# haotianteng/Chiron

Hardware: AMD Instinct MI355X
Metric: kilobases/sec basecalled (DNA_default seg_len=400 batch=1100) (higher is better)
Workload: dtype f32; 1 GPU; DNA_default seg_len=400 jump=390 batch=1100 greedy, synthetic 4 kHz signal (BASELINE.json configs[1]); segment_len=400, jump=390, batch=1100, decode=greedy, weights=seeded synthetic (exact checkpoint shapes), parallelism=reads sharded per GPU, no collective, slots_in_flight=3, parallelism_bookkeeping=none (one rank), distinct_devices=1

## Files before the change

chiron_amd/csrc/engine.hip:

```cpp
#include <hip/hip_runtime.h>

#include <algorithm>
#include <atomic>
#include <chrono>
#include <cfloat>
#include <cmath>
#include <cstdarg>
#include <cstdio>
#include <cstring>
#include <cstdlib>
#include <map>
#include <mutex>
#include <string>
#include <vector>

#include "../../include/chiron_amd.h"
#include "kernels.h"
#include "model_layout.h"
#include "weight_pack.h"
#include <dlfcn.h>

static const char* const kProfNames[] = {"conv_dma", "lstm_proj_dma", "lstm_recurrence", "fc_head", "ctc_greedy", "ctc_beam", "sparse_build",
                                         "path_prob", "conv_lift", "conv_res", "conv1_pwl", "conv_wino", "lstm_proj0_dma", "conv2a"};

// ... 63 lines not shown
};
struct CalibCtx {
  double* dev_sums = nullptr;
  size_t max_records = 0;
  std::vector<CalibRecord> rec;
  int skipped = 0;
};

struct ProfEvent {
  int name_id;
  hipEvent_t a, b;
  double flops, bytes;
};

struct Slot {
  hipStream_t stream = nullptr;
  unsigned long long* tile_ctr = nullptr;
  unsigned long long tile_base = 0;
  unsigned long long tile_base32 = 0;
  float* sig = nullptr;
  int32_t* seq = nullptr;
  float* act[5] = {nullptr, nullptr, nullptr, nullptr, nullptr};
  double* bn_sums = nullptr;
  float* z = nullptr;
  float* lasth[2] = {nullptr, nullptr};
  float* lasth_f32 = nullptr;
  float* logits = nullptr;
  uint8_t* labels = nullptr;
  int32_t* count = nullptr;
  float* log_prob = nullptr;
  float* prob = nullptr;
  int64_t* offsets = nullptr;
  int64_t* indices = nullptr;
  int64_t* values = nullptr;
  int64_t* meta = nullptr;
  void* beam_ws = nullptr;
  size_t beam_ws_bytes = 0;
  float* h_sig = nullptr;
  int32_t* h_seq = nullptr;
  int64_t* h_indices = nullptr;
  int64_t* h_values = nullptr;
  int64_t* h_meta = nullptr;
  float* h_log_prob = nullptr;
  float* h_prob = nullptr;
  float* h_logits = nullptr;
  uint8_t* h_labels = nullptr;
  int32_t* h_count = nullptr;
  uint8_t* h_flat = nullptr;
  struct State {
    std::atomic<int> v{0};
    State() {}
    State(const State& o) : v(o.v.load()) {}
    State& operator=(const State& o) {
      v.store(o.v.load());
      return *this;
    }
  } state;
  int batch = 0;
  uint32_t flags = 0;
  const float* sig_used = nullptr;
  int net_batch = 0;
  const float* rnn_out = nullptr;
  bool rnn_out_f32 = true;
  std::vector<ProfEvent> events;
  struct ScoreBufs {
    int32_t* labels = nullptr;
    int32_t* label_len = nullptr;
    float* loss = nullptr;
    float* edit = nullptr;
    int32_t* status = nullptr;
    uint64_t* ws = nullptr;
    size_t cap_labels = 0, cap_rows = 0, cap_ws = 0;
  } score;
};

struct chiron_engine : NetPlans {
  chiron_model_desc desc;
  BlobMap map;
  chiron_engine_opts opts;
  int L = 0, H = 0, K = 0;
  int maxB = 0, BP = 0;
  bool stream32 = true;
  bool stream16 = true;
  bool dyn_tiles = true;
  int lstm16_pair = -1;
  bool lstm16_fused = false;
  bool lstm16_narrow = false;
  bool lstm_fixed_roles = false;
  int lstm_form = 0;
  bool lstm_paired = false;
  bool bn_batch = false;
  bool f16 = false;
  bool w2 = false;
  bool lasth32 = true;
  bool w2_zf16 = false;
  bool split = false;
  int lasth_ld = 0;
  int kq = GEMM_BK;
  std::vector<Slot> slots;
  std::map<const float*, PlanHost> plan_host;
  std::vector<float> host_weights;
  CalibCtx* calib = nullptr;
  int calibrated = 0;
  std::vector<void*> owned;
  bool profiling = false;
  std::vector<std::string> prof_names;
  std::mutex mu;
};

static chiron_status dev_alloc(chiron_engine* e, void** p, size_t bytes, bool zero) {
  HIP_TRY(hipMalloc(p, bytes ? bytes : 16));
  e->owned.push_back(*p);
  if (zero) HIP_TRY(hipMemset(*p, 0, bytes ? bytes : 16));
  return CHIRON_OK;
}
static chiron_status upload_plans(chiron_engine* e, std::vector<Upload>& ups) {
  for (Upload& u : ups) {
    chiron_status st = dev_alloc(e, u.dst, u.bytes, false);
    if (st) return st;
    HIP_TRY(hipMemcpy(*u.dst, u.data, u.bytes, hipMemcpyHostToDevice));
    u.owner.reset();
    if (u.host.Npad > 0) e->plan_host[(const float*)*u.dst] = std::move(u.host);
  }
  return CHIRON_OK;
}

static bool split_row_scale() {
  static const bool on = getenv("CHIRON_SPLIT_NO_ROW_SCALE") == nullptr;
  return on;
}

static chiron_status build_plans(chiron_engine* e, const float* w) {
  e->bn_batch = e->desc.bn_mode == CHIRON_BN_BATCH;
  PackSwitches sw;
  sw.no_winograd = getenv("CHIRON_NO_WINOGRAD") != nullptr;
  sw.wino_f2 = getenv("CHIRON_WINOGRAD_F2") != nullptr;
  sw.wino_f4 = getenv("CHIRON_WINOGRAD_F4") != nullptr;
  sw.no_pwl = getenv("CHIRON_NO_PWL") != nullptr;
  sw.split_rec32 = getenv("CHIRON_SPLIT_REC32") != nullptr;
  if (e->split) sw.split_row_scale = split_row_scale();
  std::vector<Upload> ups;
  const chiron_status st = pack_weights(e->desc, e->map, w, e->L, e->opts.dtype, sw, e, &ups);
  return st ? st : upload_plans(e, ups);
}

static const uint64_t TENSOR_LIMIT = 0xFFFE0000ull;

static chiron_status plan_sizes(const chiron_model_desc* d, const chiron_engine_opts* o, chiron_engine_sizes* out) {
  BlobMap map;
  chiron_status st = blob_map(d, &map);
  if (st) return st;
  if (!o) return fail(CHIRON_ERR_INVALID, "null opts");
  if (o->max_batch < 1 || o->segment_len < 1) return fail(CHIRON_ERR_INVALID, "max_batch/segment_len must be positive");
  if (o->dtype != CHIRON_F32 && o->dtype != CHIRON_F16 && o->dtype != CHIRON_F32_SPLIT && o->dtype != CHIRON_F16_W2)
    return fail(CHIRON_ERR_INVALID, "dtype %d unknown (0 = f32, 1 = f16, 2 = f32 as hi/lo half pairs, 3 = f16 activations against hi/lo weights)", o->dtype);
  if (o->max_beam < 0) return fail(CHIRON_ERR_INVALID, "max_beam %d", o->max_beam);
  const bool f16 = o->dtype == CHIRON_F16 || o->dtype == CHIRON_F16_W2, split = o->dtype == CHIRON_F32_SPLIT, bn_batch = d->bn_mode == CHIRON_BN_BATCH;
  const uint64_t B = (uint64_t)o->max_batch, BP = (uint64_t)roundup(o->max_batch, 16), L = (uint64_t)o->segment_len, H = d->hidden, K = d->classes;
  SiteFrames fr[MAX_SITES];
  const uint64_t T = (uint64_t)frames(map, o->segment_len, fr);
  uint64_t tmax = 0, cmax = 0;
  for (int i = map.has_stem; i < map.n_sites; ++i) {
    tmax = std::max<uint64_t>(tmax, (uint64_t)std::max(fr[i].tin, fr[i].tout));
    cmax = std::max<uint64_t>(cmax, (uint64_t)map.site[i].co);
  }
  const uint64_t lasth_ld = !split ? 2 * H : d->rnn_kind == CHIRON_RNN_MULTI ? 2 * (uint64_t)roundup(d->hidden, 32) : (uint64_t)roundup(2 * d->hidden, 32);
  const uint64_t act = B * tmax * cmax * (f16 ? 2 : 4), lasth = T * BP * lasth_ld * 4, z = T * BP * 2 * 4 * H * 4;
  if (B * tmax >= (1ull << 31) || T * BP >= (1ull << 31))
    return fail(CHIRON_ERR_OVERFLOW, "max_batch %d x %llu frames does not fit the kernels' int row index", o->max_batch, (unsigned long long)tmax);
  if (act > TENSOR_LIMIT)
    return fail(CHIRON_ERR_OVERFLOW, "max_batch %d: an activation tensor [%d x %llu x %llu] needs %llu bytes, the kernels address at most %llu "
                "per tensor (about %llu windows at this segment length and dtype): use a smaller max_batch",
                o->max_batch, o->max_batch, (unsigned long long)tmax, (unsigned long long)cmax, (unsigned long long)act,
                (unsigned long long)TENSOR_LIMIT, (unsigned long long)(TENSOR_LIMIT / (tmax * cmax * (f16 ? 2 : 4))));
  if (T * BP * lasth_ld * (f16 ? 2 : 4) > TENSOR_LIMIT)
    return fail(CHIRON_ERR_OVERFLOW, "max_batch %d: the recurrent output [%llu x %llu x %llu] needs %llu bytes, the kernels address at most %llu per tensor",
                o->max_batch, (unsigned long long)T, (unsigned long long)BP, (unsigned long long)lasth_ld, (unsigned long long)lasth,
                (unsigned long long)TENSOR_LIMIT);
  uint64_t slot = B * L * 4 + BP * 4 + (bn_batch ? 5 : 3) * act + (bn_batch ? 2 * 2 * cmax * 8 : 0) + z + 2 * lasth + (split ? T * BP * 2 * H * 4 : 0);
  slot += B * T * K * 4 + B * T + 3 * B * 4 + (B + 1) * 8 + B * T * 16 + B * T * 8 + 3 * 8;
  if (o->max_beam > 0) slot += beam_workspace_bytes((int)B, (int)T, o->max_beam);
  if (out) {
    out->T = (int32_t)T;
    out->ratio = (double)o->segment_len / (double)T;
    out->largest_tensor_bytes = std::max(act, T * BP * lasth_ld * (f16 ? 2 : 4));
    out->tensor_limit_bytes = TENSOR_LIMIT;
    out->slot_bytes = slot;
    out->total_bytes = slot * (uint64_t)std::max(1, o->n_slots);
  }
  return CHIRON_OK;
}

extern "C" chiron_status chiron_engine_plan(const chiron_model_desc* desc, const chiron_engine_opts* opts, chiron_engine_sizes* out) {
  if (!out) return fail(CHIRON_ERR_INVALID, "null out");
  memset(out, 0, sizeof(*out));
  return plan_sizes(desc, opts, out);
}

static chiron_status alloc_slot(chiron_engine* e, Slot* s) {
  HIP_TRY(hipStreamCreateWithFlags(&s->stream, hipStreamNonBlocking));
  const size_t B = e->maxB, BP = e->BP, L = e->L, T = e->T, H = e->H, K = e->K;
  size_t tmax = 0, cmax = 0;
  for (const BlockPlan& b : e->blocks) {
    tmax = std::max<size_t>(tmax, b.t_in);
    tmax = std::max<size_t>(tmax, b.t_out);
    cmax = std::max<size_t>(cmax, b.c);
  }
  chiron_status st;
  if ((st = dev_alloc(e, (void**)&s->tile_ctr, 16 * sizeof(unsigned long long), true))) return st;
  if ((st = dev_alloc(e, (void**)&s->sig, B * L * 4, true))) return st;
  if ((st = dev_alloc(e, (void**)&s->seq, BP * 4, true))) return st;
  for (int i = 0; i < (e->bn_batch ? 5 : 3); ++i)
    if ((st = dev_alloc(e, (void**)&s->act[i], B * tmax * cmax * (e->f16 ? 2 : 4), false))) return st;
  if (e->bn_batch && (st = dev_alloc(e, (void**)&s->bn_sums, 2 * 2 * cmax * sizeof(double), true))) return st;
  if ((st = dev_alloc(e, (void**)&s->z, (size_t)T * BP * 2 * 4 * H * 4, true))) return st;
  for (int i = 0; i < 2; ++i)
    if ((st = dev_alloc(e, (void**)&s->lasth[i], T * BP * (size_t)e->lasth_ld * 4, true))) return st;
  if (e->split && (st = dev_alloc(e, (void**)&s->lasth_f32, T * BP * 2 * H * 4, true))) return st;
  if ((st = dev_alloc(e, (void**)&s->logits, B * T * K * 4, false))) return st;
  if ((st = dev_alloc(e, (void**)&s->labels, B * T, false))) return st;
  if ((st = dev_alloc(e, (void**)&s->count, B * 4, true))) return st;
  if ((st = dev_alloc(e, (void**)&s->log_prob, B * 4, true))) return st;
  if ((st = dev_alloc(e, (void**)&s->prob, B * 4, true))) return st;
  if ((st = dev_alloc(e, (void**)&s->offsets, (B + 1) * 8, true))) return st;
  if ((st = dev_alloc(e, (void**)&s->indices, B * T * 16, false))) return st;
  if ((st = dev_alloc(e, (void**)&s->values, B * T * 8, false))) return st;
  if ((st = dev_alloc(e, (void**)&s->meta, 3 * 8, true))) return st;
  if (e->opts.max_beam > 0) {
    s->beam_ws_bytes = beam_workspace_bytes((int)B, (int)T, e->opts.max_beam);
    if ((st = dev_alloc(e, &s->beam_ws, s->beam_ws_bytes, false))) return st;
  }
  HIP_TRY(hipHostMalloc((void**)&s->h_sig, B * L * 4, hipHostMallocDefault));
  HIP_TRY(hipHostMalloc((void**)&s->h_seq, BP * 4, hipHostMallocDefault));
  HIP_TRY(hipHostMalloc((void**)&s->h_indices, B * T * 16, hipHostMallocDefault));
  HIP_TRY(hipHostMalloc((void**)&s->h_values, B * T * 8, hipHostMallocDefault));
  HIP_TRY(hipHostMalloc((void**)&s->h_meta, 3 * 8, hipHostMallocDefault));
  HIP_TRY(hipHostMalloc((void**)&s->h_log_prob, B * 4, hipHostMallocDefault));
  HIP_TRY(hipHostMalloc((void**)&s->h_prob, B * 4, hipHostMallocDefault));
  HIP_TRY(hipHostMalloc((void**)&s->h_logits, B * T * K * 4, hipHostMallocDefault));
  HIP_TRY(hipHostMalloc((void**)&s->h_labels, B * T, hipHostMallocDefault));
  HIP_TRY(hipHostMalloc((void**)&s->h_count, B * 4, hipHostMallocDefault));
  s->h_flat = (uint8_t*)malloc(B * T ? B * T : 1);
  if (!s->h_flat) return fail(CHIRON_ERR_DEVICE, "out of host memory");
  memset(s->h_prob, 0, B * 4);
  return CHIRON_OK;
}

extern "C" chiron_status chiron_engine_create(const chiron_model_desc* desc, const float* weights, size_t n_floats,
                                              const chiron_engine_opts* opts, chiron_engine** out) {
  if (!out) return fail(CHIRON_ERR_INVALID, "null out");
  *out = nullptr;
  BlobMap map;
  chiron_status st = blob_map(desc, &map);
  if (st) return st;
  if (!weights || !opts) return fail(CHIRON_ERR_INVALID, "null weights/opts");
  if (map.total != n_floats) return fail(CHIRON_ERR_INVALID, "weight blob has %zu floats, descriptor needs %zu", n_floats, map.total);
  {
    chiron_engine_sizes sz;
    if ((st = plan_sizes(desc, opts, &sz))) return st;
  }
  if (desc->hidden != 100) return fail(CHIRON_ERR_INVALID, "hidden=%d: the recurrence kernel is built for hidden=100 (both shipped models)", desc->hidden);
  const bool trace = getenv("CHIRON_TRACE_CREATE") != nullptr;
  auto now = [] { return std::chrono::duration<double, std::milli>(std::chrono::steady_clock::now().time_since_epoch()).count(); };
  const double t_enter = now();
  int ndev = 0;
  if (hipGetDeviceCount(&ndev) != hipSuccess || ndev < 1) return fail(CHIRON_ERR_DEVICE, "no HIP device visible: libchiron_amd has no CPU fallback");
  if (opts->device_id < 0 || opts->device_id >= ndev) return fail(CHIRON_ERR_INVALID, "device_id %d out of range (%d devices)", opts->device_id, ndev);
  HIP_TRY(hipSetDevice(opts->device_id));
  if (trace) HIP_TRY(hipFree(nullptr));
  const double t_runtime = now();

  chiron_engine* e = new chiron_engine();
  e->desc = *desc;
  e->map = map;
  e->opts = *opts;
  if (e->opts.n_slots < 1) e->opts.n_slots = 1;
  e->L = opts->segment_len;
  e->H = desc->hidden;
  e->K = desc->classes;
  e->maxB = opts->max_batch;
  e->BP = roundup(opts->max_batch, 16);
  e->w2 = opts->dtype == CHIRON_F16_W2;
  e->w2_zf16 = e->w2 && getenv("CHIRON_W2_ZF16") != nullptr;
  e->lasth32 = getenv("CHIRON_F16_LASTH16") == nullptr;
  e->f16 = opts->dtype == CHIRON_F16 || e->w2;
  e->split = opts->dtype == CHIRON_F32_SPLIT;
  e->kq = e->f16 ? 2 * GEMM_BK : GEMM_BK;
  e->lasth_ld = !e->split ? 2 * desc->hidden
                : desc->rnn_kind == CHIRON_RNN_MULTI ? 2 * roundup(desc->hidden, 32) : roundup(2 * desc->hidden, 32);
  e->lstm_paired = getenv("CHIRON_LSTM_PAIR") != nullptr;
  e->lstm_fixed_roles = getenv("CHIRON_LSTM_FIXED_ROLES") != nullptr;
  {
    const char* wv = getenv("CHIRON_LSTM_WIDE");
    e->lstm_form = wv ? atoi(wv) : (e->split ? 0 : CHIRON_LSTM_WIDE_DEFAULT);
    if (e->lstm_form < 0 || e->lstm_form > 2) e->lstm_form = CHIRON_LSTM_WIDE_DEFAULT;
  }
  e->lstm16_narrow = getenv("CHIRON_LSTM16_NARROW") != nullptr;
  e->lstm16_pair = getenv("CHIRON_LSTM16_PAIR") ? atoi(getenv("CHIRON_LSTM16_PAIR")) : -1;
  e->stream16 = getenv("CHIRON_NO_STREAM16") == nullptr && opts->dtype != CHIRON_F16_W2;
  e->stream32 = getenv("CHIRON_NO_STREAM32") == nullptr;
  e->dyn_tiles = getenv("CHIRON_STATIC_TILES") == nullptr;
  {
    const int min_groups = getenv("CHIRON_LSTM16_FUSED_MIN") ? atoi(getenv("CHIRON_LSTM16_FUSED_MIN")) : 64;
    e->lstm16_fused = e->f16 && !e->w2 && !e->lstm16_narrow && desc->hidden == 100 && (e->BP / 16) * 2 >= min_groups && getenv("CHIRON_LSTM16_UNFUSED") == nullptr;
  }
  if (e->f16 && !e->w2) e->host_weights.assign(weights, weights + n_floats);
  st = build_plans(e, weights);
  const double t_plans = now();
  if (st == CHIRON_OK) {
    e->slots.resize(e->opts.n_slots);
    for (Slot& s : e->slots)
      if ((st = alloc_slot(e, &s))) break;
  }
  const double t_slots = now();
  if (st == CHIRON_OK && hipDeviceSynchronize() != hipSuccess) st = fail(CHIRON_ERR_DEVICE, "device sync after setup failed");
  if (trace)
    fprintf(stderr, "chiron_engine_create: {\"hip_runtime_and_context_ms\": %.1f, \"weights_prepared_and_uploaded_ms\": %.1f, \"slot_buffers_ms\": %.1f, "
                    "\"final_sync_ms\": %.1f, \"slots\": %d}\n", t_runtime - t_enter, t_plans - t_runtime, t_slots - t_plans, now() - t_slots, e->opts.n_slots);
  if (st) {
    chiron_engine_destroy(e);
    return st;
  }
  e->prof_names.assign(std::begin(kProfNames), std::end(kProfNames));
  *out = e;
  return CHIRON_OK;
}

extern "C" void chiron_engine_destroy(chiron_engine* e) {
  if (!e) return;
  hipSetDevice(e->opts.device_id);
  hipDeviceSynchronize();
  for (Slot& s : e->slots) {
    for (ProfEvent& ev : s.events) {
      hipEventDestroy(ev.a);
      hipEventDestroy(ev.b);
    }
    if (s.stream) hipStreamDestroy(s.stream);
    void* sp[] = {s.score.labels, s.score.label_len, s.score.loss, s.score.edit, s.score.status, s.score.ws};
    for (void* q : sp)
      if (q) hipFree(q);
    void* hp[] = {s.h_sig, s.h_seq, s.h_indices, s.h_values, s.h_meta, s.h_log_prob, s.h_prob, s.h_logits, s.h_labels, s.h_count};
    free(s.h_flat);
    for (void* q : hp)
      if (q) hipHostFree(q);
  }
  for (void* q : e->owned) hipFree(q);
  delete e;
}

extern "C" chiron_status chiron_engine_dims(const chiron_engine* e, int32_t* out_T, double* out_ratio) {
  if (!e) return fail(CHIRON_ERR_INVALID, "null engine");
  if (out_T) *out_T = e->T;
  if (out_ratio) *out_ratio = (double)e->L / (double)e->T;
  return CHIRON_OK;
}

enum { PN_CONV = 0, PN_PROJ, PN_REC, PN_FC, PN_GREEDY, PN_BEAM, PN_SPARSE, PN_PATHPROB, PN_LIFT, PN_RES, PN_PWL, PN_WINO, PN_PROJ0, PN_CONV2A };

struct Roctx {
  int (*push)(const char*) = nullptr;
  int (*pop)() = nullptr;
  Roctx() {
    const char* v = getenv("CHIRON_ROCTX");
    if (!v || !*v || *v == '0') return;
    for (const char* name : {"librocprofiler-sdk-roctx.so", "librocprofiler-sdk-roctx.so.1", "libroctx64.so", "libroctx64.so.4"}) {
      void* h = dlopen(name, RTLD_NOW | RTLD_GLOBAL);
      if (!h) continue;
      push = reinterpret_cast<int (*)(const char*)>(dlsym(h, "roctxRangePushA"));
      pop = reinterpret_cast<int (*)()>(dlsym(h, "roctxRangePop"));
      if (push && pop) return;
      push = nullptr, pop = nullptr;
    }
    fprintf(stderr, "chiron_amd: CHIRON_ROCTX is set but no roctx library could be loaded: no ranges\n");
  }
};
static const Roctx& roctx() {
  static const Roctx r;
  return r;
}

struct Prof {
  chiron_engine* e;
  Slot* s;
// ... 194 lines not shown
        done_pwl = launch_pwl_conv(q, s->stream);
      }
      if (!done_pwl) {
        {
          Prof pr(e, s, PN_LIFT, 2.0 * B * b.t_in * b.c, 4.0 * B * b.t_in + (e->f16 ? 2.0 : 4.0) * B * b.t_in * b.c);
          launch_lift(sig, b.lift_a, b.lift_b, bufA, (long)B * b.t_in, b.c, e->f16 ? 1 : e->split ? 2 : 0, s->stream);
        }
        GemmParams g = gemm_desc(e, b.gb, B, Mout, b.t_out, in_taps, 1, bufB, b.c);
        Prof pr(e, s, PN_CONV, 2.0 * B * b.t_out * (double)b.k * b.c * b.c, (e->f16 ? 2.0 : 4.0) * B * (b.t_in + b.t_out) * b.c);
        ok &= launch(e, g, s->stream);
      }
      GemmParams g = gemm_desc(e, b.gc, B, Mout, b.t_out, {GemmSeg{bufB, b.c, 0, b.c, cop, b.t_out, 1, 0, 0}}, 1, bufA, b.c);
      g.sig = sig;
      g.L = e->L;
      g.res_a = b.res_a;
      g.res_b = b.res_b;
      g.res_stride = b.stride;
      {
        Prof pr(e, s, PN_RES, 2.0 * B * b.t_out * (double)b.c * b.c, 8.0 * B * b.t_out * b.c);
        ok &= launch(e, g, s->stream);
      }
      x = bufA;
      xi = ia;
    } else {
      const int cip = roundup(b.c_in, e->kq);
      GemmParams g = gemm_desc(e, b.ga, B, (long)B * b.t_in, b.t_in, {GemmSeg{x, b.c_in, 0, b.c_in, cip, b.t_in, 1, 0, 0}}, 1, bufA, b.c);
      {
        Prof pr(e, s, PN_CONV2A, 2.0 * B * b.t_in * (double)b.c_in * b.c, 4.0 * B * b.t_in * (b.c_in + b.c));
        ok &= launch(e, g, s->stream);
      }
      g = gemm_desc(e, b.gb, B, Mout, b.t_out, in_taps, 1, bufB, b.c);
      {
        bool done = false;
        if (b.wino_u != nullptr) {
          WinoParams wq;
          wq.src = bufA, wq.U = b.wino_u, wq.shift = b.gb.shift, wq.out = bufB;
          wq.B = B, wq.T = b.t_in, wq.C = b.c, wq.N = b.c, wq.lda = b.c, wq.ldo = b.c, wq.relu = 1, wq.f4 = b.wino_f4;
          wq.tile_ctr = e->dyn_tiles ? s->tile_ctr : nullptr, wq.tile_base = 0, wq.tile_base_host = &s->tile_base;
          Prof pr(e, s, PN_WINO, 2.0 * B * b.t_out * (double)b.k * b.c * b.c, 4.0 * B * (b.t_in + b.t_out) * b.c);
          done = launch_wino_conv3(wq, s->stream);
        }
        if (!done) {
          Prof pr(e, s, PN_CONV, 2.0 * B * b.t_out * (double)b.k * b.c * b.c, 4.0 * B * (b.t_in + b.t_out) * b.c);
          ok &= launch(e, g, s->stream);
        }
      }
      g = gemm_desc(e, b.gc, B, Mout, b.t_out,
                    {GemmSeg{bufB, b.c, 0, b.c, cop, b.t_out, 1, 0, 0}, GemmSeg{x, b.c_in, 0, b.c_in, cip, b.t_in, b.stride, 0, 0}}, 1, bufA, b.c);
      {
        Prof pr(e, s, PN_CONV, 2.0 * B * b.t_out * (double)(b.c + b.c_in) * b.c, 4.0 * B * b.t_out * (2.0 * b.c + b.c_in));
        ok &= launch(e, g, s->stream);
      }
      x = bufA;
      xi = ia;
    }
  }
  s->sig_used = x;
  return ok;
}

static bool run_rnn(chiron_engine* e, Slot* s, int B) {
  bool ok = true;
  bool last_out_f32 = false;
  const float* fea = s->sig_used;
  const int T = e->T, H = e->H, BP = e->BP;
  const int zc = 4 * H;
  const float* prev = nullptr;
  for (size_t l = 0; l < e->lstm.size(); ++l) {
    const LstmPlan& lp = e->lstm[l];
    float* outbuf = s->lasth[l & 1];
    const bool fused = e->lstm16_fused && lp.wxwide != nullptr;
    for (int pj = 0; pj < (fused ? 0 : lp.nproj); ++pj) {
      const int Kp = roundup(lp.in_w, e->kq);
      const GemmSeg src = l == 0           ? GemmSeg{fea, e->C, 0, e->C, Kp, T, 1, 0, 0}
                          : lp.nproj == 1 ? GemmSeg{prev, e->lasth_ld, 0, 2 * H, Kp, T, 1, 0, 1}
                                          : GemmSeg{prev, e->lasth_ld, e->split ? pj * roundup(H, 32) : pj * H, H, Kp, T, 1, 0, 1};
      GemmParams g = gemm_desc(e, lp.proj[pj], B, (long)T * BP, T, {src}, 0, s->z, 0);
      g.m_time_major = 1;
      g.out_mode = 1;
      g.z_cols = zc;
      g.z_ndir = lp.nproj == 1 ? 2 : 1;
      g.z_dir0 = lp.nproj == 1 ? 0 : pj;
      g.z_seq_len = s->seq;
      g.z_f16 = (e->f16 && (!e->w2 || e->w2_zf16)) ? 1 : 0;
      const double ndir = lp.nproj == 1 ? 2.0 : 1.0;
      Prof pr(e, s, l == 0 ? PN_PROJ0 : PN_PROJ, 2.0 * B * T * (double)lp.in_w * 4 * H * ndir, 4.0 * B * T * (lp.in_w + ndir * zc));
      ok &= launch(e, g, s->stream);
    }
    LstmParams r;
    r.z = s->z;
    r.wfrag = lp.wfrag;
    r.wlight = lp.wlight;
    r.wwide = lp.wwide;
    r.wwide32 = lp.wwide32;
    r.wsplit = lp.wsplit;
    r.form32 = e->lstm_form;
    r.narrow16 = e->lstm16_narrow ? 1 : 0;
    r.xsrc = nullptr;
    r.wxwide = nullptr;
    r.whfused = nullptr;
    r.fused_pair = 0;
    r.xbias = nullptr;
    r.xK = r.xld = r.x_time_major = 0;
    if (fused) {
      r.xsrc = l == 0 ? (const void*)fea : (const void*)prev;
      r.wxwide = lp.wxwide;
      r.whfused = lp.whfused;
      r.fused_pair = e->lstm16_pair >= 0 ? (e->lstm16_pair ? 1 : 0) : ((BP / 16) * 2 > current_device_cus() ? 1 : 0);
      r.xbias = lp.proj[0].shift;
      r.xK = lp.in_w;
      r.xld = l == 0 ? e->C : e->lasth_ld;
      r.x_time_major = l == 0 ? 0 : 1;
    }
    r.seq_len = s->seq;
    r.out = e->split ? s->lasth_f32 : outbuf;
    r.out_f32 = (e->f16 && e->lasth32 && e->calib == nullptr && l + 1 == e->lstm.size()) ? 1 : 0;
    last_out_f32 = r.out_f32 != 0;
    const bool direct_split = e->split && lp.wsplit != nullptr && l + 1 < e->lstm.size();
    r.out_split = direct_split ? (void*)outbuf : nullptr;
    r.split_ld = e->lasth_ld;
    r.split_bw0 = e->desc.rnn_kind == CHIRON_RNN_MULTI ? roundup(H, 32) : H;
    r.T = T;
    r.B = B;
    r.BP = BP;
    r.H = H;
    r.ndir = 2;
    r.paired = e->lstm_paired ? 1 : 0;
    r.fixed_roles = e->lstm_fixed_roles ? 1 : 0;
    r.group0 = 0;
    r.f16 = e->f16 ? 1 : 0;
    r.w2 = e->w2 ? (e->w2_zf16 ? 2 : 1) : 0;
    if (e->calib && e->f16) {
      for (int pj = 0; pj < lp.nproj; ++pj) {
        const int dir = lp.nproj == 1 ? -1 : pj;
        if (l == 0)
          calib_measure(e, lp.proj[pj].shift, 0, fea, (long)B * T, e->C, 0, e->C, 0, B, (int)l, dir, 0, s->stream);
        else
          calib_measure(e, lp.proj[pj].shift, 0, prev, (long)T * BP, e->lasth_ld, lp.nproj == 1 ? 0 : pj * H, lp.in_w, BP, B, (int)l, dir, 0, s->stream);
      }
    }
    {
      Prof pr(e, s, PN_REC, 2.0 * 2.0 * B * T * (double)H * 4 * H + (fused ? 2.0 * B * T * (double)lp.in_w * 4 * H * 2.0 : 0.0),
              fused ? (e->f16 ? 2.0 : 4.0) * B * T * (2.0 * lp.in_w + 2.0 * H) : 4.0 * B * T * 2.0 * (zc + H));
      launch_lstm(r, s->stream);
    }
    if (e->calib && e->f16)
      for (int dir = 0; dir < 2; ++dir)
        calib_measure(e, lp.proj[lp.nproj == 1 ? 0 : dir].shift, 0, outbuf, (long)T * BP, e->lasth_ld, dir * H, H, BP, B, (int)l, dir, 1, s->stream);
    prev = outbuf;
    if (e->split) {
      if (direct_split) {
      } else if (l + 1 < e->lstm.size()) {
        Prof pr(e, s, PN_REC, 0.0, (4.0 + 4.0) * T * BP * 2.0 * H);
        const bool multi = e->desc.rnn_kind == CHIRON_RNN_MULTI;
        launch_split_convert(s->lasth_f32, outbuf, (long)T * BP, 2 * H, e->lasth_ld, multi ? H : 0, multi ? roundup(H, 32) : 0, s->stream);
      } else {
        prev = s->lasth_f32;
      }
    }
  }
  s->rnn_out = prev;
  FcParams f;
  f.lasth = prev;
  f.w = e->fc_w;
  f.bias = e->fc_b;
  f.wc = e->fc_wc;
// ... 582 lines not shown
```

chiron_amd/csrc/gemm.hip:

```cpp
#include "kernels.h"
#include "timing_variants.h"

#include <cstdlib>
#include <type_traits>

namespace chiron {

typedef float f32x16 __attribute__((ext_vector_type(16)));
typedef float f32x4 __attribute__((ext_vector_type(4)));
typedef _Float16 f16x8 __attribute__((ext_vector_type(8)));
typedef _Float16 f16x4 __attribute__((ext_vector_type(4)));

constexpr int LDS_LD = GEMM_BK + 4;
constexpr int TILE_F = GEMM_BM * LDS_LD;

struct ZGroup {
  unsigned base;
  unsigned per_t;
  int t, l0, l1, l2, l3;
  __device__ __forceinline__ ZGroup(const GemmParams& p, int t_, int b) : t(t_) {
    per_t = (unsigned)(p.BP >> 2) * p.z_dirs_total * p.z_cols * 4;
    base = (unsigned)(b >> 2) * p.z_dirs_total * p.z_cols * 4;
    const int4 len = *reinterpret_cast<const int4*>(p.z_seq_len + b);
    l0 = min(len.x, p.T_out), l1 = min(len.y, p.T_out), l2 = min(len.z, p.T_out), l3 = min(len.w, p.T_out);
// ... 826 lines not shown
#pragma unroll
              for (int j = 0; j < 4; ++j)
                if (g * 4 + j < NP) piece(g * 4 + j);
              continue;
            }
            f32x4 a[NMI], b[NNI];
#pragma unroll
            for (int mi = 0; mi < NMI; ++mi) a[mi] = *reinterpret_cast<const f32x4*>(a0 + mi * 32 * GEMM_BK + fsl(g));
#pragma unroll
            for (int ni = 0; ni < NNI; ++ni) b[ni] = *reinterpret_cast<const f32x4*>(b0 + ni * 32 * GEMM_BK + fsl(g));
            if (F16) {
#pragma unroll
              for (int j = 0; j < 4; ++j)
                if (g * 4 + j < NP) piece(g * 4 + j);
#pragma unroll
              for (int mi = 0; mi < NMI; ++mi)
#pragma unroll
                for (int ni = 0; ni < NNI; ++ni) {
                  const f32x16 c = acc[mi][ni];
                  const f16x8 ah = __builtin_bit_cast(f16x8, a[mi]), bh = __builtin_bit_cast(f16x8, b[ni]);
                  acc[mi][ni] = ZOUT ? __builtin_amdgcn_mfma_f32_32x32x16_f16(ah, bh, c, 0, 0, 0)
                                     : __builtin_amdgcn_mfma_f32_32x32x16_f16(bh, ah, c, 0, 0, 0);
                }
            } else {
#pragma unroll
              for (int j = 0; j < 4; ++j) {
                if (g * 4 + j < NP) piece(g * 4 + j);
#pragma unroll
                for (int mi = 0; mi < NMI; ++mi)
#pragma unroll
                  for (int ni = 0; ni < NNI; ++ni) {
                    const f32x16 c = acc[mi][ni];
#if CHIRON_SENS & 16
                    if (j & 1) { acc[mi][ni][0] += a[mi][j] * b[ni][j]; continue; }
#endif
                    acc[mi][ni] = ZOUT ? __builtin_amdgcn_mfma_f32_32x32x2f32(a[mi][j], b[ni][j], c, 0, 0, 0)
                                       : __builtin_amdgcn_mfma_f32_32x32x2f32(b[ni][j], a[mi][j], c, 0, 0, 0);
                  }
              }
#if CHIRON_SENS & 4096
              if (ZOUT && FS && have_prev && C * 4 + g < 4 * NNI) {
                const int sq = (C * 4 + g) / NNI, sni = (C * 4 + g) % NNI;
                const unsigned gstr = (unsigned)p.z_dirs_total * p.z_cols * 4;
                float* o = p.out + (unsigned)((pm0 + wave * 32 + 8 * sq + 4 * kh) >> 2) * gstr + (unsigned)(p.z_dir0 * p.z_cols + pn0 + li) * 4 + sni * 128;
                if (pm0 + wave * 32 + 8 * sq + 4 * kh < p.M) *reinterpret_cast<f32x4*>(o) = a[0];
              }
#endif
            }
          }
          }
        }
        buf ^= 1;
      };
      chunk(std::integral_constant<int, 0>{});
      if (CPS > 1) chunk(std::integral_constant<int, 1>{});
      if (CPS > 2) chunk(std::integral_constant<int, 2>{});
      if (CPS > 3) chunk(std::integral_constant<int, 3>{});
      if (CPS > 4) chunk(std::integral_constant<int, 4>{});
      if (CPS > 5) chunk(std::integral_constant<int, 5>{});
      if (CPS > 6) chunk(std::integral_constant<int, 6>{});
      if (CPS > 7) chunk(std::integral_constant<int, 7>{});
    };
    segment(std::true_type{}, 0);
    for (int sgi = 1; sgi < nseg; ++sgi) segment(std::false_type{}, sgi);

    have_prev = true;
    pm0 = m0;
    pn0 = n0;
    c_id = n_id;
#if CHIRON_SENS & 1024
    ++clk_tiles;
#endif
  }
  if (have_prev) epilogue(pm0, pn0);
#if CHIRON_SENS & 1024
  if (tid == 0 && blockIdx.x < 4 && clk_tiles > 0)
    printf("gemm_clk zout %d K %d block %d: tiles %llu, cycles per tile: total %llu, epilogue %llu, barriers %llu %llu %llu %llu %llu %llu %llu %llu\n",
           (int)ZOUT, p.K, (int)blockIdx.x, clk_tiles, (__builtin_amdgcn_s_memtime() - clk_t0) / clk_tiles, clk_epi / clk_tiles, clk_bar[0] / clk_tiles,
           clk_bar[1] / clk_tiles, clk_bar[2] / clk_tiles, clk_bar[3] / clk_tiles, clk_bar[4] / clk_tiles, clk_bar[5] / clk_tiles, clk_bar[6] / clk_tiles,
           clk_bar[7] / clk_tiles);
#endif
}

template <bool ZOUT, bool RES>
static bool launch_dma(const GemmParams& p, dim3 grid, dim3 block, hipStream_t stream) {
  const int kpad = p.seg[0].kpad, cin = p.seg[0].cin;
  constexpr int BN = ZOUT ? 160 : GEMM_BN;
  if (((p.N + BN - 1) / BN) * BN > DMA_MAX_N) return false;
  if (ZOUT && p.z_cols < BN) return false;
  for (int s = 1; s < p.nseg; ++s)
    if (p.seg[s].kpad != kpad || p.seg[s].cin != cin) return false;
  const bool tail = cin != kpad;
  if (p.f16 == 2) {
    if (!ZOUT && p.N % GEMM_BN) return false;
    if constexpr (ZOUT) {
      if (p.nseg == 1 && kpad == 256 && !tail) {
        hipLaunchKernelGGL((gemm_f32_dma_kernel<true, false, 8, false, 2, true>), grid, block, 0, stream, p);
        return true;
      }
      if (p.nseg == 1 && kpad == 224 && tail) {
        hipLaunchKernelGGL((gemm_f32_dma_kernel<true, false, 7, true, 2, true>), grid, block, 0, stream, p);
        return true;
      }
    }
    if (kpad == 256 && !tail) {
      hipLaunchKernelGGL((gemm_f32_dma_kernel<ZOUT, RES, 8, false, 2>), grid, block, 0, stream, p);
      return true;
    }
    if constexpr (ZOUT) {
      if (kpad == 224 && tail) {
        hipLaunchKernelGGL((gemm_f32_dma_kernel<true, false, 7, true, 2>), grid, block, 0, stream, p);
        return true;
      }
      if (kpad == 128 && tail) {
        hipLaunchKernelGGL((gemm_f32_dma_kernel<true, false, 4, true, 2>), grid, block, 0, stream, p);
        return true;
      }
    }
    return false;
  }
  if (p.f16) {
    if (!ZOUT && p.N % GEMM_BN) return false;
    if (kpad == 128 && !tail) {
      hipLaunchKernelGGL((gemm_f32_dma_kernel<ZOUT, RES, 4, false, 1>), grid, block, 0, stream, p);
      return true;
    }
    if constexpr (ZOUT) {
      if (kpad == 128 && tail) {
        hipLaunchKernelGGL((gemm_f32_dma_kernel<true, false, 4, true, 1>), grid, block, 0, stream, p);
        return true;
      }
      if (kpad == 64 && tail) {
        hipLaunchKernelGGL((gemm_f32_dma_kernel<true, false, 2, true, 1>), grid, block, 0, stream, p);
        return true;
      }
    }
    return false;
  }
  if constexpr (ZOUT) {
    if (p.nseg == 1) {
      if (kpad == 256 && !tail) {
        hipLaunchKernelGGL((gemm_f32_dma_kernel<true, false, 8, false, 0, true>), grid, block, 0, stream, p);
        return true;
      }
      if (kpad == 224 && tail) {
        hipLaunchKernelGGL((gemm_f32_dma_kernel<true, false, 7, true, 0, true>), grid, block, 0, stream, p);
        return true;
      }
    }
  }
  if (kpad == 256 && !tail) {
    hipLaunchKernelGGL((gemm_f32_dma_kernel<ZOUT, RES, 8, false>), grid, block, 0, stream, p);
    return true;
  }
  if constexpr (ZOUT) {
    if (kpad == 224 && tail) {
      hipLaunchKernelGGL((gemm_f32_dma_kernel<true, false, 7, true>), grid, block, 0, stream, p);
      return true;
    }
    if (kpad == 128 && tail) {
      hipLaunchKernelGGL((gemm_f32_dma_kernel<true, false, 4, true>), grid, block, 0, stream, p);
      return true;
    }
  }
  return false;
}

bool launch_gemm(const GemmParams& p0, hipStream_t stream) {
  GemmParams p = p0;
  const int nblocks_n = (p.N + GEMM_BN - 1) / GEMM_BN;
  const int mblocks = (p.M + GEMM_BM - 1) / GEMM_BM;
  const int total_ids = ((mblocks + 7) / 8) * 8 * nblocks_n;
  const int n_cu = current_device_cus();
  static const int wgs_per_cu = [] {
    const char* v = getenv("CHIRON_GEMM_WGS_PER_CU");
    const int n = v ? atoi(v) : 2;
    return n >= 1 && n <= 8 ? n : 2;
  }();
  int g = wgs_per_cu * n_cu;
  g = (g / 8) * 8;
  if (g > total_ids) g = total_ids;
  const dim3 grid(g), block(256);
  const int total_z = ((mblocks + 7) / 8) * 8 * ((p.N + 159) / 160);
  const dim3 grid_z(std::min((wgs_per_cu * n_cu / 8) * 8, total_z));
  const bool zout = p.out_mode == 1;
  const bool dyn = p.tile_ctr != nullptr && p.tile_base_host != nullptr && p.seg[0].src != nullptr && p.seg[0].kpad / GEMM_BK >= 3 &&
                   (zout ? grid_z.x : grid.x) % 8 == 0;
  if (dyn) p.tile_base = *p.tile_base_host;
  else p.tile_ctr = nullptr;
  auto advance = [&](bool launched) {
    if (launched && dyn) *p.tile_base_host += (unsigned long long)((zout ? total_z : total_ids) / 8 + (zout ? grid_z.x : grid.x) / 8);
    return launched;
  };
  if (p.f16) {
    if (p.seg[0].src == nullptr) return false;
    if (p.out_mode == 1) return advance(launch_dma<true, false>(p, grid_z, block, stream));
    if (p.res_a != nullptr) return advance(launch_dma<false, true>(p, grid, block, stream));
    return advance(launch_dma<false, false>(p, grid, block, stream));
  }
  if (p.seg[0].src == nullptr) {
    hipLaunchKernelGGL((gemm_f32_kernel<true, false, false>), grid, block, 0, stream, p);
  } else if (p.out_mode == 1) {
    if (!advance(launch_dma<true, false>(p, grid_z, block, stream)))
      hipLaunchKernelGGL((gemm_f32_kernel<false, true, false>), grid, block, 0, stream, p);
  } else if (p.res_a != nullptr) {
    if (!advance(launch_dma<false, true>(p, grid, block, stream)))
      hipLaunchKernelGGL((gemm_f32_kernel<false, false, true>), grid, block, 0, stream, p);
  } else {
    if (!advance(launch_dma<false, false>(p, grid, block, stream)))
      hipLaunchKernelGGL((gemm_f32_kernel<false, false, false>), grid, block, 0, stream, p);
  }
  return true;
}

}
```

chiron_amd/csrc/kernels.h:

```cpp
#pragma once
#include <hip/hip_runtime.h>
#include <stdint.h>

#include "../../include/chiron_amd.h"

#define CHIRON_KMAX 5

namespace chiron {

constexpr int CHIRON_MAX_DEVICES = 64;
inline int current_device_index() {
  int dev = 0;
  if (hipGetDevice(&dev) != hipSuccess || dev < 0 || dev >= CHIRON_MAX_DEVICES) dev = 0;
  return dev;
}
inline int current_device_cus() {
  static int n_cu[CHIRON_MAX_DEVICES] = {};
  const int dev = current_device_index();
  int n = __atomic_load_n(&n_cu[dev], __ATOMIC_RELAXED);
  if (n == 0) {
    hipDeviceProp_t prop;
    n = hipGetDeviceProperties(&prop, dev) == hipSuccess ? prop.multiProcessorCount : 0;
    if (n <= 0) n = 256;
    __atomic_store_n(&n_cu[dev], n, __ATOMIC_RELAXED);
  }
  return n;
}

constexpr int GEMM_MAX_SEG = 16;
constexpr int GEMM_BM = 128;
constexpr int GEMM_BN = 128;
constexpr int GEMM_BK = 32;

struct GemmSeg {
  const float* src;
  int lda;
  int col0;
  int cin;
  int kpad;
  int w_in;
  int stride;
  int shift;
  int time_major;
};

struct GemmParams {
  int M;
  int T_out;
  int B;
  int BP;
  int m_time_major;
  int N;
  int K;
  int nseg;
  GemmSeg seg[GEMM_MAX_SEG];
  const float* Wt;
  const float* shift;
  const float* descale;
  int relu;
  const float* sig;
  int L;
  const float* lift_a;
  const float* lift_b;
  const float* res_a;
  const float* res_b;
  int res_stride;
  float* out;
  int ldo;
  int out_mode;
  int z_cols;
  int z_ndir;
  int z_dir0;
  int z_dirs_total;
  const int32_t* z_seq_len;
  int f16;
  int z_f16;
  unsigned long long* tile_ctr;
  unsigned long long tile_base;
  unsigned long long* tile_base_host;
};

bool launch_gemm(const GemmParams& p, hipStream_t stream);
bool launch_stream16(const GemmParams& p, hipStream_t stream);
bool launch_stream32(const GemmParams& p, hipStream_t stream);


struct WinoParams {
  const float* src;
  const float* U;
  const float* shift;
  float* out;
  int B, T, C, N, lda, ldo, relu;
  int f4;
  unsigned long long* tile_ctr;
  unsigned long long tile_base;
  unsigned long long* tile_base_host;
};
bool launch_wino_conv3(const WinoParams& p, hipStream_t stream);

constexpr int LSTM_K = 100;
constexpr int LSTM_NW = 7;

struct LstmParams {
  const float* z;
  const float* wfrag;
  const float* wlight;
  const float* wwide32;
  int out_f32;
  const void* wsplit;
  void* out_split;
  int split_ld;
  int split_bw0;
  int form32;
  const void* wwide;
  const void* xsrc;
  const void* wxwide;
  const void* whfused;
  int fused_pair;
  const float* xbias;
  int xK, xld, x_time_major;
  const int32_t* seq_len;
  float* out;
  int T, B, BP, H;
  int ndir;
  int paired;
  int fixed_roles;
  int group0;
  int narrow16;
  int w2;
  int f16;
};
void launch_lstm(const LstmParams& p, hipStream_t stream);
constexpr int LSTM_KSTEPS16 = 25;

void launch_stem_conv(const float* sig, const float* w, const float* shift, void* out, int B, int L, int T_out, int k, int stride, int left,
                      int C, int fmt, int relu, hipStream_t stream);
void launch_split_convert(const float* src, void* dst, long rows, int cols, int ld, int half, int half_dst, hipStream_t stream);
struct PwlConvParams {
  const float* sig;
  const float* bp;
  const float* ref;
// ... 193 lines not shown
```

chiron_amd/csrc/weight_pack.h:

```cpp
#pragma once
#include <algorithm>
#include <cfloat>
#include <cmath>
#include <memory>
#include <utility>
#include <vector>

#include "kernels.h"
#include "model_layout.h"

namespace chiron {

inline int roundup(int v, int m) { return (v + m - 1) / m * m; }

struct ConvGemmPlan {
  float* Wt = nullptr;
  float* shift = nullptr;
  float* descale = nullptr;
  int N = 0, Npad = 0, K = 0;
};

struct PlanHost {
  std::vector<float> dW;
  std::vector<float> shift0;
  int N = 0, Npad = 0, K = 0;
};

struct BlockPlan {
  bool lift = false;
  int c_in = 0, c = 0, k = 0, stride = 1, left = 0;
  int t_in = 0, t_out = 0;
  float *lift_a = nullptr, *lift_b = nullptr;
  float *res_a = nullptr, *res_b = nullptr;
  float *pwl_bp = nullptr, *pwl_ref = nullptr, *pwl_tab = nullptr, *pwl_shift = nullptr;
  int pwl_nbp = 0;
  ConvGemmPlan ga, gb, gc;
  float* wino_u = nullptr;
  int wino_f4 = 0;
  ConvGemmPlan g1;
  bool i_bn = false;
  float *bn_scale[4] = {nullptr, nullptr, nullptr, nullptr}, *bn_offset[4] = {nullptr, nullptr, nullptr, nullptr};
};

struct LstmPlan {
  int in_w = 0;
  ConvGemmPlan proj[2];
  int nproj = 1;
  float* wfrag = nullptr;
  void* wwide = nullptr;
  void* whfused = nullptr;
  void* wxwide = nullptr;
  int wx_ksteps = 0;
  void* wsplit = nullptr;
  float* wwide32 = nullptr;
  float* wlight = nullptr;
};

struct NetPlans {
  int T = 0, C = 0;
  int stem_k = 0, stem_stride = 1, stem_left = 0, stem_t = 0, stem_c = 0;
  float *stem_w = nullptr, *stem_shift = nullptr, *stem_scale = nullptr, *stem_offset = nullptr;
  std::vector<BlockPlan> blocks;
  std::vector<LstmPlan> lstm;
  float *fc_w = nullptr, *fc_b = nullptr, *fc_wc = nullptr, *fc_bc = nullptr;
};

struct PackSwitches {
  bool no_winograd = false;
  bool wino_f2 = false;
  bool wino_f4 = false;
  bool no_pwl = false;
  bool split_rec32 = false;
  bool split_row_scale = true;
};

struct Upload {
  void** dst;
  std::shared_ptr<void> owner;
  const void* data;
  size_t bytes;
  PlanHost host;
};


struct HalfPair {
  _Float16 hi, lo;
};
inline HalfPair split_half(float v) {
  const _Float16 hi = (_Float16)v;
  return {hi, (_Float16)(v - (float)hi)};
}

struct BnFold {
  std::vector<float> inv, sh;
};
inline BnFold fold_bn(const float* scale, const float* offset, const float* mean, const float* var, int n) {
  BnFold f;
  f.inv.resize(n);
  f.sh.resize(n);
  for (int i = 0; i < n; ++i) {
    const float inv = (1.0f / sqrtf(var[i] + 1e-5f)) * scale[i];
    f.inv[i] = inv;
    f.sh[i] = offset[i] - mean[i] * inv;
  }
  return f;
}

inline void fold_filter(std::vector<float>& Wt, std::vector<float>& shift, int K, int k0, const float* W, int taps, int ci, int co, int cop,
                        const float* inv, const float* sh) {
  for (int n = 0; n < co; ++n) {
    for (int tap = 0; tap < taps; ++tap)
      for (int c = 0; c < ci; ++c) {
        const float v = W[((size_t)tap * ci + c) * co + n];
        Wt[(size_t)n * K + k0 + tap * cop + c] = inv ? v * inv[n] : v;
      }
    if (sh) shift[n] = k0 == 0 ? sh[n] : shift[n] + sh[n];
  }
}

struct LstmKernels {
  const float* kern[2];
  int H;
  float at(int dir, int k_off, int width, int k, int g, int unit) const {
    return k < width && unit < H ? kern[dir][(size_t)(k_off + k) * 4 * H + g * H + unit] : 0.f;
  }
};

template <class Put>
inline void narrow_fragments(const LstmKernels& kn, int V, int ksteps, int k_off, int width, Put put) {
  for (int dir = 0; dir < 2; ++dir)
    for (int wv = 0; wv < LSTM_NW; ++wv)
      for (int ks = 0; ks < ksteps; ++ks)
        for (int lane = 0; lane < 64; ++lane)
          for (int q = 0; q < V; ++q) {
            const int k = V * ks + q, g = lane >> 4, unit = 16 * wv + (lane & 15);
            put(((((size_t)dir * LSTM_NW + wv) * ksteps + ks) * 64 + lane) * V + q, kn.at(dir, k_off, width, k, g, unit));
          }
}
inline size_t narrow_elems(int V, int ksteps) { return (size_t)2 * LSTM_NW * ksteps * 64 * V; }

template <class Put>
inline void wide_fragments(const LstmKernels& kn, int V, int ksteps, int k_off, int width, Put put) {
  for (int dir = 0; dir < 2; ++dir)
    for (int wv = 0; wv < 8; ++wv)
      for (int slot = 0; slot < (wv == 7 ? 4 : 3); ++slot)
        for (int ks = 0; ks < ksteps; ++ks)
          for (int lane = 0; lane < 64; ++lane)
            for (int q = 0; q < V; ++q) {
              const int k = V * (4 * ks + (lane >> 4)) + q, g = lane & 3, unit = 4 * (3 * wv + slot) + ((lane >> 2) & 3);
              put((((((size_t)dir * 8 + wv) * 4 + slot) * ksteps + ks) * 64 + lane) * V + q, kn.at(dir, k_off, width, k, g, unit));
            }
}
inline size_t wide_elems(int V, int ksteps) { return (size_t)2 * 8 * 4 * ksteps * 64 * V; }

inline std::vector<float> light_fragment(const LstmKernels& kn, int k_off) {
  std::vector<float> wl((size_t)2 * 28 * 64, 0.f);
  for (int dir = 0; dir < 2; ++dir)
    for (int m = 0; m < 28; ++m)
      for (int lane = 0; lane < 64; ++lane) {
        const int q = m >> 2, a = m & 3, kg = lane >> 4, g = (lane >> 2) & 3, j = lane & 3;
        const int k = 16 * q + 4 * kg + a;
        wl[((size_t)dir * 28 + m) * 64 + lane] = kn.at(dir, k_off, kn.H, k, g, 96 + j);
      }
  return wl;
}

struct WeightPacker {
  const chiron_model_desc& d;
  const BlobMap& map;
  const float* w;
  const PackSwitches sw;
  const bool f16, w2, split, batch;
  const int kq;
// ... 328 lines not shown
```

Baseline: 4582 kbases/s.

## Run fp32 LSTM input projections as three-way bf16 split MFMA GEMM

Adds a projection GEMM kernel that splits fp32 activations and weights into hi/mid/lo bf16 planes. It accumulates six of the nine cross products with bf16 MFMA instructions, keeping fp32-level accuracy while using matrix cores instead of fp32 math. Weights are pre-split and laid out per tile on the host at setup. The kernel is used by default for the bidirectional f32 projections with 256 or 200 inputs. It costs extra LDS, weight memory and split ALU work per stage, and dropping the three smallest terms slightly changes the rounding.

Result: faster. 4832 kbases/s, median of 6 (+5.5%).

```diff
diff --git a/chiron_amd/csrc/engine.hip b/chiron_amd/csrc/engine.hip
--- a/chiron_amd/csrc/engine.hip
+++ b/chiron_amd/csrc/engine.hip
@@ -169,6 +169,7 @@
   int maxB = 0, BP = 0;
   bool stream32 = true;
   bool stream16 = true;
+  bool proj_bf16 = true;
   bool dyn_tiles = true;
   int lstm16_pair = -1;
   bool lstm16_fused = false;
@@ -227,8 +228,21 @@
   sw.split_rec32 = getenv("CHIRON_SPLIT_REC32") != nullptr;
   if (e->split) sw.split_row_scale = split_row_scale();
   std::vector<Upload> ups;
-  const chiron_status st = pack_weights(e->desc, e->map, w, e->L, e->opts.dtype, sw, e, &ups);
-  return st ? st : upload_plans(e, ups);
+  chiron_status st = pack_weights(e->desc, e->map, w, e->L, e->opts.dtype, sw, e, &ups);
+  if (st) return st;
+  if (e->proj_bf16 && e->opts.dtype == CHIRON_F32 && !e->bn_batch) {
+    for (LstmPlan& lp : e->lstm) {
+      ConvGemmPlan& g = lp.proj[0];
+      if (lp.nproj != 1 || (lp.in_w != 256 && lp.in_w != 200) || g.N % BF3_BN != 0) continue;
+      for (const Upload& u : ups) {
+        if (u.dst != reinterpret_cast<void**>(&g.Wt)) continue;
+        const std::vector<uint16_t> planes = bf16x3_planes(static_cast<const float*>(u.data), g.N, g.K, lp.in_w);
+        if ((st = dev_alloc(e, &g.w_bf3, planes.size() * sizeof(uint16_t), false))) return st;
+        HIP_TRY(hipMemcpy(g.w_bf3, planes.data(), planes.size() * sizeof(uint16_t), hipMemcpyHostToDevice));
+      }
+    }
+  }
+  return upload_plans(e, ups);
 }
 
 static const uint64_t TENSOR_LIMIT = 0xFFFE0000ull;
@@ -386,6 +400,7 @@
   e->lstm16_pair = getenv("CHIRON_LSTM16_PAIR") ? atoi(getenv("CHIRON_LSTM16_PAIR")) : -1;
   e->stream16 = getenv("CHIRON_NO_STREAM16") == nullptr && opts->dtype != CHIRON_F16_W2;
   e->stream32 = getenv("CHIRON_NO_STREAM32") == nullptr;
+  e->proj_bf16 = getenv("CHIRON_PROJ_FP32") == nullptr;
   e->dyn_tiles = getenv("CHIRON_STATIC_TILES") == nullptr;
   {
     const int min_groups = getenv("CHIRON_LSTM16_FUSED_MIN") ? atoi(getenv("CHIRON_LSTM16_FUSED_MIN")) : 64;
@@ -746,6 +761,7 @@
       g.z_ndir = lp.nproj == 1 ? 2 : 1;
       g.z_dir0 = lp.nproj == 1 ? 0 : pj;
       g.z_seq_len = s->seq;
+      g.w_bf3 = lp.proj[pj].w_bf3;
       g.z_f16 = (e->f16 && (!e->w2 || e->w2_zf16)) ? 1 : 0;
       const double ndir = lp.nproj == 1 ? 2.0 : 1.0;
       Prof pr(e, s, l == 0 ? PN_PROJ0 : PN_PROJ, 2.0 * B * T * (double)lp.in_w * 4 * H * ndir, 4.0 * B * T * (lp.in_w + ndir * zc));
diff --git a/chiron_amd/csrc/gemm.hip b/chiron_amd/csrc/gemm.hip
--- a/chiron_amd/csrc/gemm.hip
+++ b/chiron_amd/csrc/gemm.hip
@@ -932,6 +932,215 @@
 #endif
 }
 
+typedef __bf16 bf16x8 __attribute__((ext_vector_type(8)));
+typedef unsigned u32x4 __attribute__((ext_vector_type(4)));
+constexpr int BF3_TERMS = 6;
+constexpr bool BF3_SMALL_FIRST = true;
+
+__device__ __forceinline__ void bf3_split(const f32x4& x0, const f32x4& x1, bf16x8& h, bf16x8& m, bf16x8& l) {
+  unsigned hb[8], mb[8], lb[8];
+#pragma unroll
+  for (int e = 0; e < 8; ++e) {
+    const float x = e < 4 ? x0[e] : x1[e - 4];
+    hb[e] = __builtin_bit_cast(unsigned, x);
+    const float r = x - __builtin_bit_cast(float, hb[e] & 0xffff0000u);
+    mb[e] = __builtin_bit_cast(unsigned, r);
+    lb[e] = __builtin_bit_cast(unsigned, r - __builtin_bit_cast(float, mb[e] & 0xffff0000u));
+  }
+  u32x4 hp, mp, lp;
+#pragma unroll
+  for (int i = 0; i < 4; ++i) {
+    hp[i] = __builtin_amdgcn_perm(hb[2 * i + 1], hb[2 * i], 0x07060302u);
+    mp[i] = __builtin_amdgcn_perm(mb[2 * i + 1], mb[2 * i], 0x07060302u);
+    lp[i] = __builtin_amdgcn_perm(lb[2 * i + 1], lb[2 * i], 0x07060302u);
+  }
+  h = __builtin_bit_cast(bf16x8, hp);
+  m = __builtin_bit_cast(bf16x8, mp);
+  l = __builtin_bit_cast(bf16x8, lp);
+}
+
+template <int NST, bool TAIL>
+__global__ __launch_bounds__(256, 2) void gemm_proj_bf16x3_kernel(const GemmParams p) {
+  constexpr int BN = BF3_BN, NNI = 5;
+  constexpr int A_F = GEMM_BM * BF3_BK;
+  constexpr int B_F = BF3_STAGE_BYTES / 4;
+  constexpr int B_PIECES = BF3_STAGE_BYTES / 1024;
+  __shared__ __attribute__((aligned(16))) float lds[2 * A_F + 2 * B_F + DMA_MAX_N];
+  float* const As = lds;
+  float* const Bs = As + 2 * A_F;
+  float* const shl = Bs + 2 * B_F;
+
+  const int tid = threadIdx.x;
+  if (p.K < 0) lds[tid] = 0.f;
+  for (int n = tid; n < DMA_MAX_N; n += 256) shl[n] = n < p.N ? p.shift[n] : 0.f;
+  const int lane = tid & 63;
+  const int wave = __builtin_amdgcn_readfirstlane(tid >> 6);
+  const int li = lane & 31;
+  const int kh = lane >> 5;
+
+  const int nblocks_n = p.N / BN;
+  const int mblocks = (p.M + GEMM_BM - 1) / GEMM_BM;
+  const int total_ids = ((mblocks + 7) / 8) * 8 * nblocks_n;
+
+  auto tile_of = [&](int id, int& m0, int& n0) -> bool {
+    const int xcd = id & 7;
+    const int slot = id >> 3;
+    const int mblk = (slot / nblocks_n) * 8 + xcd;
+    m0 = mblk * GEMM_BM;
+    n0 = (slot % nblocks_n) * BN;
+    return mblk < mblocks;
+  };
+  auto next_valid = [&](int id) -> int {
+    int m0, n0;
+    do id += gridDim.x;
+    while (id < total_ids && !tile_of(id, m0, n0));
+    return id;
+  };
+
+  const int arow = wave * 32 + (lane >> 2);
+  const int alog = ((lane & 3) ^ ((lane >> 4) & 3)) * 4;
+  const GemmSeg& sg = p.seg[0];
+  const __amdgpu_buffer_rsrc_t ra = dma_rsrc(sg.src), rb = dma_rsrc(reinterpret_cast<const float*>(p.w_bf3));
+  const unsigned blane = (unsigned)lane * 16u;
+  unsigned aoff[2];
+  unsigned btile = 0;
+  auto load_tile = [&](int id) {
+    int m0, n0;
+    tile_of(id, m0, n0);
+    const RowSplit rs(m0, p.BP);
+    btile = (unsigned)(n0 / BN) * (unsigned)(NST * BF3_STAGE_BYTES);
+#pragma unroll
+    for (int j = 0; j < 2; ++j) {
+      int t, b;
+      rs.split(arow + 16 * j, t, b);
+      const int in_t = t * sg.stride + sg.shift;
+      const bool ok = m0 + arow + 16 * j < p.M && b < p.B && in_t >= 0 && in_t < sg.w_in;
+      const long row = sg.time_major ? ((long)in_t * p.BP + b) : ((long)b * sg.w_in + in_t);
+      aoff[j] = ok ? (unsigned)((row * sg.lda + sg.col0 + alog) * 4) : DMA_OOB;
+    }
+  };
+  auto issue = [&](int c, int nb) {
+    float* const a_dst = As + nb * A_F + wave * 512;
+#pragma unroll
+    for (int j = 0; j < 2; ++j) {
+      if (TAIL && c == NST - 1) {
+        const bool ok = aoff[j] != DMA_OOB && c * BF3_BK + alog < sg.cin;
+        __builtin_amdgcn_raw_ptr_buffer_load_lds(ra, (lptr_t)(a_dst + j * 256), 16, ok ? aoff[j] + (unsigned)c * (BF3_BK * 4u) : DMA_OOB, 0, 0, 0);
+      } else {
+        __builtin_amdgcn_raw_ptr_buffer_load_lds(ra, (lptr_t)(a_dst + j * 256), 16, aoff[j], c * (BF3_BK * 4), 0, 0);
+      }
+    }
+    float* const b_dst = Bs + nb * B_F;
+#pragma unroll
+    for (int j = 0; j < (B_PIECES + 3) / 4; ++j) {
+      const int q = wave + 4 * j;
+      if (q < B_PIECES)
+        __builtin_amdgcn_raw_ptr_buffer_load_lds(rb, (lptr_t)(b_dst + q * 256), 16, blane, (int)btile + c * BF3_STAGE_BYTES + q * 1024, 0, 0);
+    }
+  };
+
+  __shared__ int sh_next;
+  const bool dyn = p.tile_ctr != nullptr;
+  const int my_xcd = blockIdx.x & 7;
+  const unsigned slots_per_xcd = (unsigned)(total_ids >> 3);
+  unsigned long long grabbed = 0;
+  auto issue_grab = [&]() {
+    if (tid == 0) grabbed = atomicAdd(p.tile_ctr + my_xcd, 1ull);
+  };
+  auto decode_grab = [&]() -> int {
+    for (;;) {
+      const unsigned long long v = grabbed - p.tile_base;
+      if (v >= slots_per_xcd) return total_ids;
+      const int id = (int)((unsigned)v << 3) | my_xcd;
+      int mm, nn;
+      if (tile_of(id, mm, nn)) return id;
+      grabbed = atomicAdd(p.tile_ctr + my_xcd, 1ull);
+    }
+  };
+  int c_id = blockIdx.x;
+  if (dyn) {
+    issue_grab();
+    if (tid == 0) sh_next = decode_grab();
+    __syncthreads();
+    c_id = sh_next;
+    if (c_id >= total_ids) return;
+  } else {
+    int m0, n0;
+    if (c_id >= total_ids) return;
+    if (!tile_of(c_id, m0, n0)) c_id = next_valid(c_id);
+    if (c_id >= total_ids) return;
+  }
+  load_tile(c_id);
+  issue(0, 0);
+  int buf = 0;
+  bool have_prev = false;
+  int pm0 = 0, pn0 = 0;
+  f32x16 acc[1][NNI];
+  const int fa = (wave * 32 + li) * BF3_BK + ((kh ^ ((li >> 2) & 3)) * 4);
+  const int fb = (kh * BN + li) * 4;
+
+  while (c_id < total_ids) {
+    int m0, n0;
+    tile_of(c_id, m0, n0);
+    int n_id = dyn ? total_ids : next_valid(c_id);
+
+    auto stage = [&](int c, auto first_tag) {
+      constexpr bool FIRST = decltype(first_tag)::value;
+      __builtin_amdgcn_s_waitcnt(0x0F70);
+      __syncthreads();
+      if (dyn) {
+        if (FIRST) issue_grab();
+        if (c == 1 && tid == 0) sh_next = decode_grab();
+        if (c == 2) n_id = sh_next;
+      }
+      if (c + 1 < NST) {
+        issue(c + 1, buf ^ 1);
+      } else if (n_id < total_ids) {
+        load_tile(n_id);
+        issue(0, buf ^ 1);
+      }
+      if (FIRST) {
+        if (have_prev) gemm_epilogue_zrows<NNI>(p, acc, pm0, pn0, wave, li, kh);
+        asm volatile("" ::: "memory");
+#pragma unroll
+        for (int ni = 0; ni < NNI; ++ni) {
+          const float sh = shl[n0 + ni * 32 + li];
+#pragma unroll
+          for (int r = 0; r < 16; ++r) acc[0][ni][r] = sh;
+        }
+      }
+      const float* const ar = As + buf * A_F + fa;
+      const float* const br = Bs + buf * B_F + fb;
+      bf16x8 ah, am, al;
+      bf3_split(*reinterpret_cast<const f32x4*>(ar), *reinterpret_cast<const f32x4*>(As + buf * A_F + (fa ^ 8)), ah, am, al);
+      bf16x8 bp[3][NNI];
+#pragma unroll
+      for (int ni = 0; ni < NNI; ++ni)
+#pragma unroll
+        for (int pl = 0; pl < 3; ++pl) bp[pl][ni] = __builtin_bit_cast(bf16x8, *reinterpret_cast<const f32x4*>(br + ni * 128 + pl * (2 * BN * 4)));
+      const bf16x8 ap[3] = {ah, am, al};
+      constexpr int TERMS[9][2] = {{2, 2}, {1, 2}, {2, 1}, {0, 2}, {1, 1}, {2, 0}, {0, 1}, {1, 0}, {0, 0}};
+#pragma unroll
+      for (int k = 0; k < BF3_TERMS; ++k) {
+        const int t = BF3_SMALL_FIRST ? k + (9 - BF3_TERMS) : 8 - k;
+#pragma unroll
+        for (int ni = 0; ni < NNI; ++ni)
+          acc[0][ni] = __builtin_amdgcn_mfma_f32_32x32x16_bf16(ap[TERMS[t][0]], bp[TERMS[t][1]][ni], acc[0][ni], 0, 0, 0);
+      }
+      buf ^= 1;
+    };
+    stage(0, std::true_type{});
+#pragma unroll 1
+    for (int c = 1; c < NST; ++c) stage(c, std::false_type{});
+
+    have_prev = true;
+    pm0 = m0;
+    pn0 = n0;
+    c_id = n_id;
+  }
+  if (have_prev) gemm_epilogue_zrows<NNI>(p, acc, pm0, pn0, wave, li, kh);
+}
+
 template <bool ZOUT, bool RES>
 static bool launch_dma(const GemmParams& p, dim3 grid, dim3 block, hipStream_t stream) {
   const int kpad = p.seg[0].kpad, cin = p.seg[0].cin;
@@ -986,6 +1195,18 @@
       }
     }
     return false;
+  }
+  if constexpr (ZOUT) {
+    if (p.nseg == 1 && p.w_bf3 != nullptr && p.N % BF3_BN == 0 && !p.z_f16) {
+      if (cin == 256) {
+        hipLaunchKernelGGL((gemm_proj_bf16x3_kernel<16, false>), grid, block, 0, stream, p);
+        return true;
+      }
+      if (cin == 200) {
+        hipLaunchKernelGGL((gemm_proj_bf16x3_kernel<13, true>), grid, block, 0, stream, p);
+        return true;
+      }
+    }
   }
   if constexpr (ZOUT) {
     if (p.nseg == 1) {
diff --git a/chiron_amd/csrc/kernels.h b/chiron_amd/csrc/kernels.h
--- a/chiron_amd/csrc/kernels.h
+++ b/chiron_amd/csrc/kernels.h
@@ -31,6 +31,9 @@
 constexpr int GEMM_BM = 128;
 constexpr int GEMM_BN = 128;
 constexpr int GEMM_BK = 32;
+constexpr int BF3_BN = 160;
+constexpr int BF3_BK = 16;
+constexpr int BF3_STAGE_BYTES = 3 * 2 * BF3_BN * 8 * 2;
 
 struct GemmSeg {
   const float* src;
@@ -57,6 +60,7 @@
   const float* Wt;
   const float* shift;
   const float* descale;
+  const void* w_bf3;
   int relu;
   const float* sig;
   int L;
diff --git a/chiron_amd/csrc/weight_pack.h b/chiron_amd/csrc/weight_pack.h
--- a/chiron_amd/csrc/weight_pack.h
+++ b/chiron_amd/csrc/weight_pack.h
@@ -2,6 +2,8 @@
 #include <algorithm>
 #include <cfloat>
 #include <cmath>
+#include <cstdint>
+#include <cstring>
 #include <memory>
 #include <utility>
 #include <vector>
@@ -17,6 +19,7 @@
   float* Wt = nullptr;
   float* shift = nullptr;
   float* descale = nullptr;
+  void* w_bf3 = nullptr;
   int N = 0, Npad = 0, K = 0;
 };
 
@@ -89,6 +92,46 @@
 inline HalfPair split_half(float v) {
   const _Float16 hi = (_Float16)v;
   return {hi, (_Float16)(v - (float)hi)};
+}
+
+struct Bf16x3 {
+  uint16_t hi, mid, lo;
+};
+inline uint32_t f32_bits(float v) {
+  uint32_t u;
+  memcpy(&u, &v, 4);
+  return u;
+}
+inline float bits_f32(uint32_t u) {
+  float v;
+  memcpy(&v, &u, 4);
+  return v;
+}
+inline Bf16x3 split_bf16x3(float w) {
+  const uint32_t hb = f32_bits(w) & 0xffff0000u;
+  const float r = w - bits_f32(hb);
+  const uint32_t mb = f32_bits(r) & 0xffff0000u;
+  const float l = r - bits_f32(mb);
+  return {(uint16_t)(hb >> 16), (uint16_t)(mb >> 16), (uint16_t)(f32_bits(l) >> 16)};
+}
+
+inline int bf16x3_stages(int cin) { return (cin + BF3_BK - 1) / BF3_BK; }
+inline size_t bf16x3_index(int plane, int n, int k, int stages) {
+  const int tile = n / BF3_BN, col = n % BF3_BN, c = k / BF3_BK, kk = k % BF3_BK;
+  const int kh = (kk >> 2) & 1, e = ((kk >> 3) << 2) | (kk & 3);
+  return ((size_t)(tile * stages + c) * (BF3_STAGE_BYTES / 2)) + (size_t)(((plane * 2 + kh) * BF3_BN + col) * 8 + e);
+}
+inline std::vector<uint16_t> bf16x3_planes(const float* Wt, int N, int ld, int cin) {
+  const int stages = bf16x3_stages(cin);
+  std::vector<uint16_t> v((size_t)(N / BF3_BN) * stages * (BF3_STAGE_BYTES / 2), (uint16_t)0);
+  for (int n = 0; n < N; ++n)
+    for (int k = 0; k < cin; ++k) {
+      const Bf16x3 s = split_bf16x3(Wt[(size_t)n * ld + k]);
+      v[bf16x3_index(0, n, k, stages)] = s.hi;
+      v[bf16x3_index(1, n, k, stages)] = s.mid;
+      v[bf16x3_index(2, n, k, stages)] = s.lo;
+    }
+  return v;
 }
 
 struct BnFold {
```
